# j-wilson/GPflowPILCO

Measured on AMD Instinct MI355X. Metric: moment_matched_rollout_step_elements_per_sec, higher is better.
Workload: dtype f32; 1 GPU; C3 (BASELINE configs[2]): N=2000 d=8 D=8 H=40 fp32 drift moment-match step / closed rollout; recipe=baseline: BASELINE.md recipe: lengthscales log-U[0.3,3], GP-prior targets, fresh mu~U[0,1]^d / Sigm~; N=2000, d=8, D=8, H=40, B_per_gpu=256, B_total=256, B_this_rank=256, parallelism=dp1 over B (weak), recipe=baseline, steps_requested=418, diag_pairs=f64, offdiag_pairs=f32

## Files before the change

gpflowpilco_amd/_lib.py:

```python
from __future__ import annotations

import ctypes as C
import os

_HERE = os.path.dirname(os.path.abspath(__file__))
LIB_PATH = os.environ.get("GPFLOWPILCO_MM_LIB") or os.path.join(_HERE, "libgpflowpilco_mm.so")

MM_F32, MM_F64 = 0, 1
MM_DMAX = 32
MM_M_ALIGN = 128
MM_FULL_OUTPUT_COV = 1
MM_MODEL_UNCERTAINTY = 2
MM_FORCE_GENERIC = 4
MM_STAGE_DIAG = 8
MM_STAGE_OFFDIAG = 16
MM_STAGE_FINALIZE = 32
MM_FORCE_WORST_TIER = 64
MM_WORKSPACE_CURRENT = 128
MM_FORCE_ROUTE = 256
MM_NO_ROUTE = 512
MM_SUMS_CURRENT = 1024

ERRORS = {
    -1: "MM_E_ARG: NULL pointer or non-positive size",
    -2: "MM_E_DIM: input dimension d exceeds MM_DMAX=32 or unsupported shape",
    -3: "MM_E_DTYPE: dtype must be MM_F32 or MM_F64",
    -4: "MM_E_WORKSPACE: workspace/packed buffer too small",
    -5: "MM_E_NO_C: model_uncertainty requested but the model was packed without C",
    -6: "MM_E_STATE: Euler update / closed rollout needs d == L and a full output covariance",
}

SIGNATURES = {
    "mm_abi_version": (C.c_int, []),
    "mm_packed_model_bytes": (C.c_size_t, [C.c_int] * 5),
    "mm_pack_model": (C.c_int, [C.c_void_p, C.c_size_t, C.c_int, C.c_int, C.c_int, C.c_int]
                      + [C.c_void_p] * 6 + [C.c_void_p]),
    "mm_pack_perm": (C.c_int, [C.c_void_p, C.c_size_t, C.c_int, C.c_int, C.c_int, C.c_int, C.c_void_p, C.c_void_p]),
    "mm_workspace_bytes": (C.c_size_t, [C.c_int] * 6),
    "mm_moment_match": (C.c_int, [C.c_void_p, C.c_size_t, C.c_int, C.c_int, C.c_int, C.c_int, C.c_int,
                                  C.c_void_p, C.c_void_p, C.c_int, C.c_double,
                                  C.c_void_p, C.c_void_p, C.c_void_p,
                                  C.c_void_p, C.c_size_t, C.c_void_p, C.c_void_p]),
    "mm_q_forward": (C.c_int, [C.c_void_p, C.c_size_t, C.c_int, C.c_int, C.c_int, C.c_int, C.c_int,
                               C.c_void_p, C.c_void_p, C.c_int,
                               C.c_void_p, C.c_void_p, C.c_void_p,
                               C.c_void_p, C.c_size_t, C.c_void_p, C.c_void_p]),
    "mm_Q_reduce_forward": (C.c_int, [C.c_void_p, C.c_size_t, C.c_int, C.c_int, C.c_int, C.c_int, C.c_int,
                                      C.c_int, C.c_double, C.c_void_p,
                                      C.c_void_p, C.c_size_t, C.c_void_p]),
    "mm_euler_update": (C.c_int, [C.c_int, C.c_int, C.c_int, C.c_double] + [C.c_void_p] * 8),
    "mm_expected_cost": (C.c_int, [C.c_int, C.c_int, C.c_int] + [C.c_void_p] * 6),
    "mm_offdiag_stats": (C.c_int, [C.c_void_p, C.c_size_t, C.c_int, C.c_int, C.c_int, C.c_int, C.c_int, C.c_int,
                                   C.c_void_p, C.c_size_t, C.c_void_p, C.c_void_p]),
    "mm_route_estimates": (C.c_int, [C.c_void_p, C.c_size_t, C.c_int, C.c_int, C.c_int, C.c_int, C.c_int, C.c_int,
                                     C.c_void_p, C.c_size_t, C.c_void_p, C.c_void_p]),
    "mm_compose_workspace_bytes": (C.c_size_t, [C.c_int] * 4),
    "mm_rollout_composed": (C.c_int, [C.c_void_p, C.c_size_t, C.c_int, C.c_int, C.c_int,
                                      C.c_void_p, C.c_size_t, C.c_int, C.c_int,
                                      C.c_int, C.c_int, C.c_int, C.c_double, C.c_int, C.c_int, C.POINTER(C.c_int32),
                                      C.c_double, C.c_double, C.c_void_p, C.c_void_p,
                                      C.c_void_p, C.c_void_p, C.c_void_p, C.c_void_p, C.c_void_p,
                                      C.c_void_p, C.c_size_t, C.c_void_p, C.c_size_t, C.c_void_p, C.c_size_t,
                                      C.c_void_p, C.c_void_p]),
    "mm_compose_nd_workspace_bytes": (C.c_size_t, [C.c_int] * 5),
    "mm_rollout_composed_nd": (C.c_int, [C.c_void_p, C.c_size_t, C.c_int, C.c_int, C.c_int,
                                         C.c_void_p, C.c_size_t, C.c_int, C.c_int,
                                         C.c_int, C.c_int, C.c_int, C.c_double, C.c_int, C.c_int, C.POINTER(C.c_int32),
                                         C.c_int, C.POINTER(C.c_double), C.POINTER(C.c_double), C.c_void_p, C.c_void_p,
                                         C.c_void_p, C.c_void_p, C.c_void_p, C.c_void_p, C.c_void_p,
                                         C.c_void_p, C.c_size_t, C.c_void_p, C.c_size_t, C.c_void_p, C.c_size_t,
                                         C.c_void_p, C.c_void_p]),
    "mm_compose_tape_bytes": (C.c_size_t, [C.c_int] * 6),
    "mm_rollout_composed_taped": (C.c_int, [C.c_void_p, C.c_size_t, C.c_int, C.c_int, C.c_int,
                                            C.c_void_p, C.c_size_t, C.c_int, C.c_int,
                                            C.c_int, C.c_int, C.c_int, C.c_double, C.c_int, C.c_int, C.POINTER(C.c_int32),
                                            C.c_double, C.c_double, C.c_void_p, C.c_void_p,
                                            C.c_void_p, C.c_void_p, C.c_void_p,
                                            C.c_void_p, C.c_size_t, C.c_void_p, C.c_size_t, C.c_void_p, C.c_size_t,
                                            C.c_void_p, C.c_void_p]),
    "mm_compose_backward_workspace_bytes": (C.c_size_t, [C.c_int] * 4),
    "mm_policy_grad_bytes": (C.c_size_t, [C.c_int] * 3),
    "mm_rollout_composed_backward": (C.c_int, [C.c_void_p, C.c_size_t, C.c_int, C.c_int, C.c_int,
                                               C.c_void_p, C.c_size_t, C.c_int, C.c_int,
                                               C.c_int, C.c_int, C.c_int, C.c_double, C.c_int, C.c_int, C.POINTER(C.c_int32),
                                               C.c_double, C.c_double, C.c_void_p, C.c_void_p,
                                               C.c_void_p, C.c_size_t, C.c_void_p,
                                               C.c_void_p, C.c_void_p, C.c_void_p,
                                               C.c_void_p, C.c_size_t, C.c_void_p, C.c_size_t,
# ... 99 lines not shown
```

gpflowpilco_amd/csrc/mm_common.h:

```cpp
#pragma once
#include <stddef.h>
#include <stdint.h>
#include "../../include/gpflowpilco_mm.h"

static inline size_t mm_align_up(size_t x, size_t a) { return (x + a - 1) / a * a; }
static inline int mm_round_up_int(int x, int a) { return (x + a - 1) / a * a; }
static inline size_t mm_elem_size(int dtype) { return dtype == MM_F64 ? 8 : 4; }

#define MM_ISTAGE_NO_ROUTE (1 << 20)
#define MM_ISTAGE_ROUTE (1 << 21)
#define MM_ISTAGE_NO_M56 (1 << 22)
#define MM_ISTAGE_OLD_OFFDIAG (1 << 23)
#define MM_ISTAGE_OLD_SPOLY56 (1 << 24)

static inline int mm_num_pairs(int L, int flags) {
  return (flags & MM_FULL_OUTPUT_COV) ? L * (L + 1) / 2 : L;
}

static inline int mm_moment_deg(int d) { return d <= 8 ? 4 : 2; }
static inline long long mm_binom(int n, int k) {
  if (k < 0 || k > n) return 0;
  long long r = 1;
  for (int i = 1; i <= k; ++i) r = r * (n - k + i) / i;
  return r;
}
static inline int mm_mono_count(int n, int d) { return (int)mm_binom(d + n - 1, n); }
static inline int mm_mono_offset(int n, int d) { int o = 0; for (int m = 0; m < n; ++m) o += mm_mono_count(m, d); return o; }
static inline size_t mm_rank_table_entries(int d) {
  const int dk = d <= 8 ? 8 : 32, deg = mm_moment_deg(d);
  size_t n = 0, p = 1;
  for (int k = 1; k <= deg; ++k) { p *= dk; n += p; }
  return n;
}
static inline int mm_moment_cols(int d) { return mm_round_up_int(mm_mono_offset(mm_moment_deg(d) + 1, d), 16); }
static inline int mm_moment56_off5(int d) { return d <= 8 ? mm_round_up_int(mm_mono_count(4, d), 128) : 0; }
static inline int mm_moment56_off6(int d) { return d <= 8 ? mm_moment56_off5(d) + mm_round_up_int(mm_mono_count(5, d), 128) : 0; }
static inline int mm_moment56_cols(int d) { return d <= 8 ? mm_moment56_off6(d) + mm_round_up_int(mm_mono_count(6, d), 128) : 0; }
struct MMTab56 { int ins[6], last[6], n_i16, mult2, mult3, n_f32; size_t bytes; };
static inline MMTab56 mm_tab56(int d) {
  MMTab56 t;
  int o = 0;
  for (int m = 0; m < 6; ++m) { t.ins[m] = o; o += mm_mono_count(m, d) * 8; }
  for (int k = 0; k < 6; ++k) { t.last[k] = o; o += mm_mono_count(k, d); }
  t.n_i16 = mm_round_up_int(o, 8);
  t.mult2 = 0; t.mult3 = mm_mono_count(2, d); t.n_f32 = mm_mono_count(2, d) + mm_mono_count(3, d);
  t.bytes = (size_t)t.n_i16 * 2 + (size_t)t.n_f32 * 4;
// ... 223 lines not shown
```

gpflowpilco_amd/csrc/mm_moments.hip:

```cpp
#include <hip/hip_runtime.h>
#include <math.h>
#include "mm_common.h"
#include "mm_mono.h"

typedef double f64x4m __attribute__((ext_vector_type(4)));

#define MM_GEMM_RB 64
#define MM_GEMM_NB 128
#define MM_GEMM_KB 32
#define MM_GEMM_AS 34
#define MM_GEMM_BS 144

__device__ __forceinline__ void mm_decode_pair_m(int p, int L, int& a, int& a2) {
  int r = p - L, i = 0;
  while (r >= L - 1 - i) { r -= L - 1 - i; ++i; }
  a = i; a2 = i + 1 + r;
}

__global__ __launch_bounds__(256) __attribute__((amdgpu_waves_per_eu(2, 2))) void k_wmom_gemm(const double* __restrict__ whR, const double* __restrict__ whC,
                                                      const double* __restrict__ Zm, int KMp, int L, int Mp, int B, int Po,
                                                      int nrb, int ncb, int nwork, int col_deg3,
                                                      const unsigned int* __restrict__ amaxc, const double* __restrict__ zmax2,
                                                      const int* __restrict__ gperm, double* __restrict__ mom) {
  const int orig = blockIdx.x;
// ... 285 lines not shown
      const int nsz = ksz >> LB;
      for (int idx = tid; idx < nsz; idx += 256) {
        double s = 0.0;
#pragma unroll
        for (int l = 0; l < DK; ++l) s = fma(cur[MM_PADI(l * nsz + idx)], dmu[l], s);
        oth[MM_PADI(idx)] = s;
      }
      __syncthreads();
      double* tsw = cur; cur = oth; oth = tsw;
      ksz = nsz;
      sign_binom = -sign_binom * (double)k / (double)(n - k + 1);
    }
    __syncthreads();
  }
  const double tot = mm_block_sum256m(total, red);
  if (tid == 0) s12[(size_t)b * Po + po] = tot + nh[0] * qh[0];
#undef MM_PADI
}

int mm_launch_wmom_full(const char* packed, const MMModelLayout& ml, char* ws, const MMWorkspaceLayout& wl,
                        int B, int L, int d, hipStream_t stream) {
  const int nrb = ((L - 1) * B + MM_GEMM_RB - 1) / MM_GEMM_RB, ncb = (ml.KMp + MM_GEMM_NB - 1) / MM_GEMM_NB;
  const long long nwork_ll = (long long)L * ncb * MM_MOM_SPLIT * nrb;
  if (nwork_ll <= 0 || nwork_ll > 0x7fffffffLL) return MM_E_DIM;
  hipLaunchKernelGGL(k_wmom_gemm, dim3((int)nwork_ll), dim3(256), 0, stream, (const double*)(ws + wl.whR),
                     (const double*)(ws + wl.whC), (const double*)(packed + ml.Zm), ml.KMp, L, wl.Mp, B, wl.Po, nrb, ncb,
                     (int)nwork_ll, 0x7fffffff , (const unsigned int*)nullptr, (const double*)(packed + ml.zmax2),
                     (const int*)nullptr, (double*)(ws + wl.mom));
  hipError_t e = hipGetLastError();
  return e == hipSuccess ? 0 : (int)e;
}

int mm_launch_moments56(const char* packed, const MMModelLayout& ml, char* ws, const MMWorkspaceLayout& wl,
                        int B, int L, int d, int allow, int old_spoly56, hipStream_t stream);

int mm_launch_moments(const char* packed, const MMModelLayout& ml, char* ws, const MMWorkspaceLayout& wl,
                      int B, int L, int d, const void* mu_f32, int flags, hipStream_t stream) {
  const double* Zm = (const double*)(packed + ml.Zm);
  double* mom = (double*)(ws + wl.mom);
  const int deg = mm_moment_deg(d) >= 4 ? 3 : mm_moment_deg(d);
  const int ncol_fwd = mm_mono_offset(deg + 1, d);
  const int nrb = ((L - 1) * B + MM_GEMM_RB - 1) / MM_GEMM_RB, ncb = (ncol_fwd + MM_GEMM_NB - 1) / MM_GEMM_NB;
  const long long nwork_ll = (long long)L * ncb * MM_MOM_SPLIT * nrb;
  if (nwork_ll <= 0 || nwork_ll > 0x7fffffffLL) return MM_E_DIM;
  const int nwork = (int)nwork_ll;
  const int allow = (flags & (MM_FORCE_WORST_TIER | MM_ISTAGE_NO_M56)) ? 0 : 1;
  const int col_deg3 = mm_mono_offset(3, d);
  const bool some = allow && mm_moment_deg(d) >= 4;
  if (some) {
    hipLaunchKernelGGL(k_wmom_perm, dim3(L), dim3(1024), 0, stream, (const unsigned int*)(ws + wl.amaxc),
                       (const double*)(packed + ml.zmax2), L, B, wl.Po, (int*)(ws + wl.gperm));
    hipError_t ep = hipGetLastError();
    if (ep != hipSuccess) return (int)ep;
  }
  hipLaunchKernelGGL(k_wmom_gemm, dim3(nwork), dim3(256), 0, stream, (const double*)(ws + wl.whR),
                     (const double*)(ws + wl.whC), Zm, ml.KMp, L, wl.Mp, B, wl.Po, nrb, ncb, nwork, col_deg3,
                     some ? (const unsigned int*)(ws + wl.amaxc) : (const unsigned int*)nullptr,
                     (const double*)(packed + ml.zmax2), some ? (const int*)(ws + wl.gperm) : (const int*)nullptr, mom);
  hipError_t e = hipGetLastError();
  if (e != hipSuccess) return (int)e;
  const int off1 = mm_mono_offset(1, d), off2 = mm_mono_offset(2, d), off3 = mm_mono_offset(3, d), off4 = mm_mono_offset(4, d);
#define MM_SPOLY(DK_, LB_)                                                                                                       \
  do {                                                                                                                          \
    const int dn_ = 1 << (LB_ * deg);                                                                                           \
    const int up_ = dn_ >> LB_;                                                                                                 \
    const size_t shm_ = (size_t)(dn_ + (dn_ >> 5) + up_ + (up_ >> 5) + 2 * ml.KMp + DK_ * DK_ + DK_ + 8) * sizeof(double);      \
    hipLaunchKernelGGL((k_spoly<DK_, LB_>), dim3(wl.Po, B), dim3(256), shm_, stream, (const double*)mom, ml.KMp,                \
                       (const double*)(ws + wl.pairmat), (const double*)(packed + ml.zbar), (const double*)(packed + ml.zmax2), \
                       (const unsigned int*)(ws + wl.amax), (const unsigned int*)(ws + wl.amaxc), (const float*)mu_f32, L, d, wl.P, deg, allow, off1, off2, off3, off4, \
                       (const short*)(packed + ml.rtab),                                                                        \
                       (double)MM_C6_C0, (double)MM_C6_C1, (double*)(ws + wl.s12));                                             \
  } while (0)
  if (d <= 8) MM_SPOLY(8, 3); else MM_SPOLY(32, 5);
#undef MM_SPOLY
  e = hipGetLastError();
  if (e != hipSuccess) return (int)e;
  if (flags & MM_ISTAGE_NO_M56) {
    if (mm_moment56_cols(d) <= 0 || wl.Po <= 0) return 0;
    const hipError_t em = hipMemsetAsync(ws + wl.s56, 0xFF, (size_t)B * wl.Po * sizeof(double), stream);
    if (em != hipSuccess) return (int)em;
    const hipError_t es = hipMemsetAsync(ws + wl.estS, 0, (size_t)B * wl.Po * sizeof(float), stream);
    return es == hipSuccess ? 0 : (int)es;
  }
  return mm_launch_moments56(packed, ml, ws, wl, B, L, d, some ? 1 : 0, (flags & MM_ISTAGE_OLD_SPOLY56) ? 1 : 0, stream);
}

__global__ void k_offdiag_stats(const unsigned int* __restrict__ amax, const double* __restrict__ zmax2,
                                const unsigned char* __restrict__ gflag, int ng, int L, int Po, int n,
                                int32_t* __restrict__ out) {
  const int idx = blockIdx.x * blockDim.x + threadIdx.x;
  bool c = false, in = false, part = false;
  int groups = 0;
  if (idx < n) {
    int a, a2;
    mm_decode_pair_m(L + idx % Po, L, a, a2);
    const float b2 = mm_collapse_bound2(amax[idx], zmax2[a2]);
    c = b2 <= MM_COLLAPSE_BOUND2;
    in = b2 <= MM_INSIDE_BOUND2;
    part = !c && mm_item_collapsed(amax[n + idx]);
    for (int g = 0; g < ng; ++g) groups += gflag[(size_t)idx * ng + g] ? 1 : 0;
  }
  const unsigned long long m = __ballot(c), mi = __ballot(in), mp = __ballot(part);
  if ((threadIdx.x & 63) == 0 && m) atomicAdd(out, (int)__popcll(m));
  if ((threadIdx.x & 63) == 0 && mi) atomicAdd(out + 2, (int)__popcll(mi));
  if ((threadIdx.x & 63) == 0 && mp) atomicAdd(out + 4, (int)__popcll(mp));
#pragma unroll
  for (int off = 32; off > 0; off >>= 1) groups += __shfl_down(groups, off, 64);
  if ((threadIdx.x & 63) == 0 && groups) atomicAdd(out + 5, groups);
  if (idx == 0) out[1] = n;
}

extern "C" int mm_offdiag_stats(const void* packed, size_t packed_bytes, int L, int M, int d, int dtype, int B, int flags,
                                const void* workspace, size_t workspace_bytes, int32_t* out, void* stream) {
  if (!packed || !workspace || !out || L <= 0 || M <= 0 || d <= 0 || d > MM_DMAX || B <= 0) return MM_E_ARG;
  const MMModelLayout ml = mm_model_layout(L, M, d, dtype, 1);
  const MMWorkspaceLayout wl = mm_workspace_layout(B, L, M, d, dtype, flags);
  if (packed_bytes < ml.Cm || workspace_bytes < wl.total) return MM_E_WORKSPACE;
// ... 16 lines not shown
```

gpflowpilco_amd/csrc/mm_moments6.hip:

```cpp
#include <hip/hip_runtime.h>
#include <math.h>
#include "mm_common.h"
#include "mm_mono.h"
#include "mm_f32_tile.h"
#include <atomic>
#include <type_traits>

__device__ __forceinline__ void mm6_decode_pair_o(int lp, int L, int& a, int& a2) {
  int r = lp, i = 0;
  while (r >= L - 1 - i) { r -= L - 1 - i; ++i; }
  a = i; a2 = i + 1 + r;
}

__global__ __launch_bounds__(256) void k_pack_zm56(char* packed, MMModelLayout lay, int L, int M, int d, int N56p,
                                                   const double* __restrict__ Z) {
  const int c = blockIdx.x, a = blockIdx.y, tid = threadIdx.x;
  const int n4 = mm_binom_i(d + 3, 4), n5 = mm_binom_i(d + 4, 5), n6 = mm_binom_i(d + 5, 6);
  const int off5 = ((n4 + 127) / 128) * 128;
  const int off6 = off5 + ((n5 + 127) / 128) * 128;
  const double* zbar = (const double*)(packed + lay.zbar) + (size_t)a * d;
  unsigned short* oh = (unsigned short*)(packed + lay.Zm56) + (((size_t)a * 2 + 0) * N56p + c) * lay.Mp;
  unsigned short* om = (unsigned short*)(packed + lay.Zm56) + (((size_t)a * 2 + 1) * N56p + c) * lay.Mp;
  int n = 0, k[6] = {0, 0, 0, 0, 0, 0};
  if (c < n4) { n = 4; mm_mono_unrank(c, 4, k); }
// ... 147 lines not shown
#pragma unroll
    for (int ks = 0; ks < 2; ++ks) {
      const int ch = ((ks * 2 + h) ^ swz) * 16;
      bf16x8 Ah[2], Am[2], Th[2], Tm[2];
#pragma unroll
      for (int t = 0; t < 2; ++t) {
        Ah[t] = *reinterpret_cast<const bf16x8*>(base + fragA[t] + ch);
        Am[t] = *reinterpret_cast<const bf16x8*>(base + 8192 + fragA[t] + ch);
        Th[t] = *reinterpret_cast<const bf16x8*>(base + fragB[t] + ch);
        Tm[t] = *reinterpret_cast<const bf16x8*>(base + 8192 + fragB[t] + ch);
      }
#pragma unroll
      for (int rt = 0; rt < 2; ++rt)
#pragma unroll
        for (int ct = 0; ct < 2; ++ct) {
          acc[rt][ct] = __builtin_amdgcn_mfma_f32_32x32x16_bf16(Am[rt], Th[ct], acc[rt][ct], 0, 0, 0);
          acc[rt][ct] = __builtin_amdgcn_mfma_f32_32x32x16_bf16(Ah[rt], Tm[ct], acc[rt][ct], 0, 0, 0);
          acc[rt][ct] = __builtin_amdgcn_mfma_f32_32x32x16_bf16(Ah[rt], Th[ct], acc[rt][ct], 0, 0, 0);
        }
    }
  }
#pragma unroll
  for (int rt = 0; rt < 2; ++rt)
#pragma unroll
    for (int e = 0; e < 16; ++e) {
      const int item = orow[wr * 64 + rt * 32 + 8 * (e >> 2) + 4 * h + (e & 3)];
      if (item < 0) continue;
      float* o = mom56 + (size_t)item * N56p + (size_t)cb * MM6_TB + wc * 64 + l31;
#pragma unroll
      for (int ct = 0; ct < 2; ++ct) o[ct * 32] = acc[rt][ct][e];
    }
}

#ifndef MM6_THREADS
#define MM6_THREADS 768
#endif
#define MM6_WAVES (MM6_THREADS / 64)
#ifndef MM6_NC
#define MM6_NC 2
#endif
template <int K, bool TRANSG, int MODE, int NC = MM6_NC, int NW = MM6_WAVES>
__device__ __forceinline__ void mm6_step(const float* __restrict__ Tin, int nJin, int nI, float* __restrict__ Tout, int nJp,
                                         const short* __restrict__ ins, int d, const float (&G)[64], const float* __restrict__ multJ,
                                         int xs, float& acc, int wave, int lane) {
  const int chunks = (nJp + 64 * NC - 1) / (64 * NC);
  auto dots = [&](auto i0c, const float (&v)[NC][8], float (&s)[NC][8]) __attribute__((always_inline)) {
    constexpr int I0 = decltype(i0c)::value;
#pragma unroll
    for (int q = 0; q < NC; ++q)
#pragma unroll
      for (int i = I0; i < 8; ++i) s[q][i] = G[0 * 8 + i] * v[q][0];
#pragma unroll
    for (int j = 1; j < 8; ++j)
#pragma unroll
      for (int q = 0; q < NC; ++q)
#pragma unroll
        for (int i = I0; i < 8; ++i) s[q][i] = fmaf(G[j * 8 + i], v[q][j], s[q][i]);
  };
  auto body = [&](int I, int t, const int (&Jp)[NC], const bool (&jv)[NC], const int (&off)[NC][8], const float (&mj)[NC]) __attribute__((always_inline)) {
    const float* tin = Tin + I * nJin;
    float v[NC][8], s[NC][8];
#pragma unroll
    for (int q = 0; q < NC; ++q)
#pragma unroll
      for (int j = 0; j < 8; ++j) v[q][j] = tin[off[q][j]];
    if (t < 4) dots(std::integral_constant<int, 0>{}, v, s);
// ... 450 lines not shown
        G[4 * q] = g4.x; G[4 * q + 1] = g4.y; G[4 * q + 2] = g4.z; G[4 * q + 3] = g4.w;
      }
    };
    float acc4 = 0.0f, dummy = 0.0f;
    const float* Q4 = nq + sy[4];
    const float* N4 = nq;
    load_G(1);
    mm6_do<D8, 0, false, 0, NC0, NW, 4, 0>(Q4, Bf4, sy, tabi, tb, d, G, nullptr, 0, dummy, wave, lane);
    __syncthreads();
    mm6_do<D8, 1, false, 1, 1, NW, 3, 37>(Bf4, X4, sy, tabi, tb, d, G, mult2, xs4, dummy, wave, lane);
    __syncthreads();
    load_G(0);
    mm6_do<D8, 0, true, 0, NC0, NW, 4, 0>(N4, Bf4, sy, tabi, tb, d, G, nullptr, 0, dummy, wave, lane);
    __syncthreads();
    mm6_do<D8, 1, true, 2, 1, NW, 3, 37>(Bf4, X4, sy, tabi, tb, d, G, nullptr, xs4, acc4, wave, lane);
    double tot = (double)MM_C6_C1 * (double)acc4;
#pragma unroll
    for (int off = 32; off > 0; off >>= 1) {
      tot += __shfl_down(tot, off, 64); s2r += __shfl_down(s2r, off, 64); s2c += __shfl_down(s2c, off, 64);
    }
    if (lane == 0) { redd[wave * 3 + 0] = tot; redd[wave * 3 + 1] = s2r; redd[wave * 3 + 2] = s2c; }
    __syncthreads();
    if (tid == 0) {
      double t = 0.0, r2 = 0.0, c2 = 0.0;
      for (int w = 0; w < NW; ++w) { t += redd[w * 3]; r2 += redd[w * 3 + 1]; c2 += redd[w * 3 + 2]; }
      s56[item] = t;
      estS[item] = mm6_estS(bound2, false, false, r2, c2);
    }
    __syncthreads();
  }
}

int mm_launch_moments56(const char* packed, const MMModelLayout& ml, char* ws, const MMWorkspaceLayout& wl,
                        int B, int L, int d, int allow, int old_spoly56, hipStream_t stream) {
  const int N56p = mm_moment56_cols(d);
  if (N56p <= 0 || wl.Po <= 0) return 0;
  if (allow) {
    const int nrb = ((L - 1) * B + MM6_TB - 1) / MM6_TB, ncb = N56p / MM6_TB;
    const long long nwork_ll = (long long)L * ncb * nrb;
    if (nwork_ll <= 0 || nwork_ll > 0x7fffffffLL) return MM_E_DIM;
    if ((size_t)B * wl.Po * 4 * wl.Mp >= 0xffffffffull || (size_t)L * 2 * N56p * wl.Mp >= 0xffffffffull) return MM_E_DIM;
    const size_t shm = 2 * MM6_STAGE_BYTES + MM6_TB * sizeof(int);
    static std::atomic<unsigned long long> attr_done{0ull};
    int dev = 0;
    if (hipGetDevice(&dev) != hipSuccess) dev = 64;
    const unsigned long long bit = (dev >= 0 && dev < 64) ? (1ull << dev) : 0ull;
    if (!bit || !(attr_done.load() & bit)) {
      const hipError_t ea = hipFuncSetAttribute((const void*)k_wmom56_gemm, hipFuncAttributeMaxDynamicSharedMemorySize, (int)shm);
      if (ea != hipSuccess) return (int)ea;
      attr_done.fetch_or(bit);
    }
    hipLaunchKernelGGL(k_wmom56_gemm, dim3((int)nwork_ll), dim3(256), shm, stream, (const unsigned short*)(ws + wl.wsp),
                       (const unsigned short*)(packed + ml.Zm56), N56p, L, wl.Mp, B, wl.Po, nrb, ncb, (int)nwork_ll,
                       mm_moment56_off5(d) / MM6_TB, mm_moment56_off6(d) / MM6_TB,
                       (const int*)(ws + wl.gperm), (float*)(ws + wl.mom56));
    hipError_t e = hipGetLastError();
    if (e != hipSuccess) return (int)e;
  }
  const int nitem = B * wl.Po;
  int* ilist = (int*)(ws + wl.ilist);
  {
    const hipError_t em = hipMemsetAsync(ilist, 0, 16, stream);
    if (em != hipSuccess) return (int)em;
  }
  hipLaunchKernelGGL(k_item_classes, dim3((nitem + 255) / 256), dim3(256), 0, stream, (const unsigned int*)(ws + wl.amaxc),
                     (const double*)(packed + ml.zmax2), L, wl.Po, nitem, allow, ilist, (double*)(ws + wl.s56), (float*)(ws + wl.estS));
  {
    const hipError_t ec = hipGetLastError();
    if (ec != hipSuccess) return (int)ec;
  }
  if (!allow) return 0;
  int sy[7];
  for (int k = 0; k < 7; ++k) sy[k] = mm_mono_count(k, d);
  size_t nfl = (size_t)2 * (sy[4] + sy[5] + sy[6]) + (size_t)sy[3] * (sy[3] + 1) + (size_t)sy[2] * sy[4] + (size_t)sy[1] * sy[5] + 6 * MM6_WAVES + 128 + 16
               + (size_t)sy[1] * sy[3] + (size_t)sy[2] * (sy[2] + 1);
  nfl = (nfl + 1) & ~(size_t)1;
  const size_t shm = nfl * sizeof(float);
  static std::atomic<unsigned long long> attr2_done{0ull};
  static std::atomic<int> ncu_cached[64];
  int dev = 0;
  if (hipGetDevice(&dev) != hipSuccess) dev = 64;
  const unsigned long long bit2 = (dev >= 0 && dev < 64) ? (1ull << dev) : 0ull;
  int ncu = bit2 ? ncu_cached[dev].load() : 0;
  if (!bit2 || !(attr2_done.load() & bit2)) {
    hipError_t ea = hipFuncSetAttribute((const void*)k_spoly56<false>, hipFuncAttributeMaxDynamicSharedMemorySize, 160 * 1024);
// ... 28 lines not shown
```

gpflowpilco_amd/csrc/mm_route.hip:

```cpp
#include <hip/hip_runtime.h>
#include <math.h>
#include "mm_common.h"
#include "mm_fork.h"
#include "mm_mono.h"
#include "mm_adjoint.h"

__device__ __forceinline__ void mmx_decode_pair_o(int lp, int L, int& a, int& a2) {
  int r = lp, i = 0;
  while (r >= L - 1 - i) { r -= L - 1 - i; ++i; }
  a = i; a2 = i + 1 + r;
}

__device__ __forceinline__ double mmx_est(double e2, unsigned int, double) {
  return 5.9604644775390625e-8 * (2.0 / 3.0) * sqrt(e2);
}

__global__ __launch_bounds__(64) void k_route_decide(const float* __restrict__ estO, int npanel, const double* __restrict__ s12,
                                                     const double* __restrict__ f1raw, const unsigned int* __restrict__ amax,
                                                     const double* __restrict__ zmax2, int L, int Po, double tol, int force,
                                                     int* __restrict__ rlist, int* __restrict__ rcount, int* __restrict__ rflag,
                                                     int slot, int32_t* __restrict__ status, const float* __restrict__ estS) {
  const int b = blockIdx.x, lane = threadIdx.x;
  auto zmax2a2 = [&](int po) { int a, a2; mmx_decode_pair_o(po, L, a, a2); return zmax2[a2]; };
  double sc = 0.0;
// ... 44 lines not shown
  for (int po = lane; po < Po; po += 64) {
    int a, a2;
    mmx_decode_pair_o(po, L, a, a2);
    const double v = fabs(s12[(size_t)b * Po + po] - f1raw[(size_t)b * L + a] * f1raw[(size_t)b * L + a2]);
    sc = v > sc ? v : sc;
  }
#pragma unroll
  for (int off = 32; off > 0; off >>= 1) { const double o = __shfl_xor(sc, off, 64); sc = o > sc ? o : sc; }
  for (int po = lane; po < Po; po += 64) {
    const float* e = estO + ((size_t)b * Po + po) * npanel;
    double e2 = 0.0;
    for (int pn = 0; pn < npanel; ++pn) e2 += (double)e[pn];
    if (estS) e2 += (double)estS[(size_t)b * Po + po];
    out[((size_t)b * Po + po) * 2 + 0] = mmx_est(e2, amax[(size_t)b * Po + po], zmax2a2(po));
    out[((size_t)b * Po + po) * 2 + 1] = sc;
  }
}

extern "C" int mm_route_estimates(const void* packed, size_t packed_bytes, int L, int M, int d, int dtype, int B, int flags,
                                  const void* workspace, size_t workspace_bytes, double* out, void* stream) {
  if (!packed || !workspace || !out || L <= 0 || M <= 0 || d <= 0 || d > MM_DMAX || B <= 0) return MM_E_ARG;
  if (dtype != MM_F32) return MM_E_DTYPE;
  const MMWorkspaceLayout wl = mm_workspace_layout(B, L, M, d, dtype, flags);
  const MMModelLayout ml = mm_model_layout(L, M, d, dtype, 1);
  if (workspace_bytes < wl.total || packed_bytes < ml.Cm) return MM_E_WORKSPACE;
  if (wl.Po <= 0) return 0;
  const char* ws = (const char*)workspace;
  if (const int rj = mm_fork_join_wait((hipStream_t)stream)) return rj;
  hipLaunchKernelGGL(k_route_report, dim3(B), dim3(64), 0, (hipStream_t)stream, (const float*)(ws + wl.estO),
                     (wl.Mp + MM_PANEL_ROWS - 1) / MM_PANEL_ROWS, (const double*)(ws + wl.s12), (const double*)(ws + wl.f1raw),
                     (const unsigned int*)(ws + wl.amax), (const double*)((const char*)packed + ml.zmax2), L, wl.Po, out,
                     d <= 8 ? (const float*)(ws + wl.estS) : (const float*)nullptr);
  hipError_t e = hipGetLastError();
  return e == hipSuccess ? 0 : (int)e;
}

__device__ __forceinline__ double mmx_rem(double x) {
  if (fabs(x) < 0.5) {
    double p = 4.7794773323873853e-14;
    p = fma(p, x, 7.6471637318198165e-13);
    p = fma(p, x, 1.1470745597729725e-11);
    p = fma(p, x, 1.6059043836821613e-10);
    p = fma(p, x, 2.08767569878681e-09);
    p = fma(p, x, 2.505210838544172e-08);
    p = fma(p, x, 2.755731922398589e-07);
    p = fma(p, x, 2.7557319223985893e-06);
    p = fma(p, x, 2.48015873015873e-05);
    p = fma(p, x, 1.984126984126984e-04);
    p = fma(p, x, 1.388888888888889e-03);
    p = fma(p, x, 8.333333333333333e-03);
    p = fma(p, x, 4.1666666666666664e-02);
    p = fma(p, x, 1.6666666666666666e-01);
    return (x * x) * (x * p);
  }
  return expm1(x) - fma(0.5 * x, x, x);
}

__device__ __forceinline__ double mmx_wave_sum(double v) {
#pragma unroll
  for (int off = 32; off > 0; off >>= 1) v += __shfl_xor(v, off, 64);
  return v;
}

template <int DK, bool AGG>
__global__ __launch_bounds__(256) void k_route_f64(const int* __restrict__ rlist, const int* __restrict__ rcount,
                                                   const double* __restrict__ Zt64, const double* __restrict__ Zc64, int Kz,
// ... 176 lines not shown
```

gpflowpilco_amd/ops.py:

```python
from __future__ import annotations

from dataclasses import dataclass, field
from typing import Dict, Optional, Tuple

import torch

from . import _lib
from ._lib import (MM_F32, MM_F64, MM_FORCE_GENERIC, MM_FULL_OUTPUT_COV, MM_WORKSPACE_CURRENT, MM_SUMS_CURRENT,
                   MM_MODEL_UNCERTAINTY, check, lib)

_DTYPES = {torch.float32: MM_F32, torch.float64: MM_F64}


def _dtype_code(dtype: torch.dtype) -> int:
  try:
    return _DTYPES[dtype]
  except KeyError:
    raise TypeError(f"moment matching supports float32/float64 states, got {dtype}") from None


def _ptr(t: Optional[torch.Tensor]):
  return None if t is None else t.data_ptr()


def _require_device(*tensors: torch.Tensor):
  for t in tensors:
    if t is not None and not t.is_cuda:
      raise RuntimeError("gpflowpilco_amd kernels run on the GPU only (no CPU fallback): "
                         f"got a tensor on {t.device}")


def _stream(device) -> int:
  return torch.cuda.current_stream(device).cuda_stream

# ... 172 lines not shown
  return c, n, inside


def offdiag_row_groups(pm: PackedModel, B: int, flags: int):
  ws = pm.workspace(B, flags, peek=True)
  out = torch.zeros(6, dtype=torch.int32, device=pm.device)
  rc = lib().mm_offdiag_stats(pm.buf.data_ptr(), pm.nbytes, pm.L, pm.M, pm.d, _dtype_code(pm.dtype), B, flags,
                              ws.data_ptr(), ws.numel(), out.data_ptr(), _stream(pm.device))
  check(rc, "mm_offdiag_stats")
  o = out.tolist()
  Mp = (pm.M + _lib.MM_M_ALIGN - 1) // _lib.MM_M_ALIGN * _lib.MM_M_ALIGN
  return o[4], o[5], o[1] * (Mp // 64)


def offdiag_routed(pm: PackedModel, B: int, flags: int) -> int:
  if pm.dtype != torch.float32 or pm.L < 2 or not (flags & MM_FULL_OUTPUT_COV):
    return 0
  ws = pm.workspace(B, flags, peek=True)
  out = torch.zeros(6, dtype=torch.int32, device=pm.device)
  rc = lib().mm_offdiag_stats(pm.buf.data_ptr(), pm.nbytes, pm.L, pm.M, pm.d, _dtype_code(pm.dtype), B, flags,
                              ws.data_ptr(), ws.numel(), out.data_ptr(), _stream(pm.device))
  check(rc, "mm_offdiag_stats")
  return int(out[3])


def route_estimates(pm: PackedModel, B: int, flags: int) -> torch.Tensor:
  Po = pm.L * (pm.L - 1) // 2 if (flags & MM_FULL_OUTPUT_COV) else 0
  out = torch.zeros(B, Po, 2, dtype=torch.float64, device=pm.device)
  if Po:
    ws = pm.workspace(B, flags, peek=True)
    rc = lib().mm_route_estimates(pm.buf.data_ptr(), pm.nbytes, pm.L, pm.M, pm.d, _dtype_code(pm.dtype), B, flags,
                                  ws.data_ptr(), ws.numel(), out.data_ptr(), _stream(pm.device))
    check(rc, "mm_route_estimates")
  return out


def euler_update(mu, Sigma, f1, Sff, cross_pre, dt: float = 1.0):
  _require_device(mu, Sigma, f1, Sff, cross_pre)
  B, d = mu.shape
  if f1.shape != (B, d) or Sff.shape != (B, d, d) or cross_pre.shape != (B, d, d):
    raise ValueError("euler_update needs d == L and a full output covariance")
  args = [t.contiguous() for t in (mu, Sigma, f1, Sff, cross_pre)]
  mu_o, S_o = torch.empty_like(args[0]), torch.empty_like(args[1])
  rc = lib().mm_euler_update(B, d, _dtype_code(mu.dtype), float(dt), *[t.data_ptr() for t in args],
                             mu_o.data_ptr(), S_o.data_ptr(), _stream(mu.device))
  check(rc, "mm_euler_update")
  return mu_o, S_o


def rollout_closed(pm: PackedModel, mu: torch.Tensor, Sigma: torch.Tensor, num_steps: int,
                   dt: float = 1.0, model_uncertainty: bool = True, jitter: float = 0.0,
                   keep_trajectory: bool = False, force_generic: bool = False):
  B, mu, Sigma = _prep_state(pm, mu, Sigma)
  mu, Sigma = mu.clone(), Sigma.clone()
  flags = make_flags(True, model_uncertainty, force_generic)
  ws = pm.workspace(B, flags)
  tmu = tS = None
  if keep_trajectory:
    tmu = torch.empty(num_steps, B, pm.d, dtype=pm.dtype, device=pm.device)
    tS = torch.empty(num_steps, B, pm.d, pm.d, dtype=pm.dtype, device=pm.device)
  rc = lib().mm_rollout_closed(pm.buf.data_ptr(), pm.nbytes, pm.L, pm.M, pm.d, _dtype_code(pm.dtype), B,
                               int(num_steps), float(dt), flags, float(jitter),
                               mu.data_ptr(), Sigma.data_ptr(), _ptr(tmu), _ptr(tS),
                               ws.data_ptr(), ws.numel(), pm.status().data_ptr(), _stream(pm.device))
  check(rc, "mm_rollout_closed")
  return (mu, Sigma, tmu, tS) if keep_trajectory else (mu, Sigma)
# ... 407 lines not shown
```

include/gpflowpilco_mm.h:

```cpp
#ifndef GPFLOWPILCO_MM_H
#define GPFLOWPILCO_MM_H

#include <stddef.h>
#include <stdint.h>

#ifdef __cplusplus
extern "C" {
#endif

#define MM_F32 0
#define MM_F64 1

#define MM_DMAX 32
#define MM_M_ALIGN 128

#define MM_FULL_OUTPUT_COV   1
#define MM_MODEL_UNCERTAINTY 2
#define MM_FORCE_GENERIC     4
#define MM_STAGE_DIAG        8
#define MM_STAGE_OFFDIAG    16
#define MM_STAGE_FINALIZE   32
#define MM_FORCE_WORST_TIER 64
#define MM_WORKSPACE_CURRENT 128
#define MM_FORCE_ROUTE 256
// ... 34 lines not shown
                    void* Sff,
                    void* cross_pre,
                    void* workspace, size_t workspace_bytes,
                    int32_t* status, void* stream);

int mm_q_forward(const void* packed, size_t packed_bytes, int L, int M, int d, int dtype, int B,
                 const void* mu, const void* Sigma, int flags,
                 void* f1, void* cross_pre, void* q_out,
                 void* workspace, size_t workspace_bytes, int32_t* status, void* stream);

int mm_Q_reduce_forward(const void* packed, size_t packed_bytes, int L, int M, int d, int dtype, int B,
                        int flags, double jitter, void* Sff,
                        void* workspace, size_t workspace_bytes, void* stream);

int mm_euler_update(int B, int d, int dtype, double dt,
                    const void* mu, const void* Sigma,
                    const void* f1, const void* Sff, const void* cross_pre,
                    void* mu_out, void* Sigma_out, void* stream);

int mm_rollout_closed(const void* packed, size_t packed_bytes, int L, int M, int d, int dtype, int B, int H,
                      double dt, int flags, double jitter,
                      void* mu, void* Sigma, void* traj_mu, void* traj_Sigma,
                      void* workspace, size_t workspace_bytes,
                      int32_t* status, void* stream);

int mm_expected_cost(int N, int d, int dtype, const void* mean, const void* cov,
                     const void* target, const void* precis, void* cost, void* stream);

int mm_offdiag_stats(const void* packed, size_t packed_bytes, int L, int M, int d, int dtype, int B, int flags,
                     const void* workspace, size_t workspace_bytes, int32_t* out, void* stream);

int mm_route_estimates(const void* packed, size_t packed_bytes, int L, int M, int d, int dtype, int B, int flags,
                       const void* workspace, size_t workspace_bytes, double* out, void* stream);

size_t mm_compose_workspace_bytes(int B, int nx, int na, int dtype);
int mm_rollout_composed(const void* drift_packed, size_t drift_bytes, int drift_L, int drift_M, int drift_d,
                        const void* policy_packed, size_t policy_bytes, int policy_M, int policy_d,
                        int dtype, int B, int H, double dt, int nx, int na, const int32_t* active_dims,
                        double head_scale, double head_shift, const void* target, const void* precis,
                        void* mx, void* Sxx, void* cost, void* traj_mu, void* traj_Sigma,
                        void* ws_drift, size_t ws_drift_bytes, void* ws_policy, size_t ws_policy_bytes,
                        void* ws_compose, size_t ws_compose_bytes, int32_t* status, void* stream);

size_t mm_compose_nd_workspace_bytes(int B, int nx, int na, int nu, int dtype);
int mm_rollout_composed_nd(const void* drift_packed, size_t drift_bytes, int drift_L, int drift_M, int drift_d,
                           const void* policy_packed, size_t policy_bytes, int policy_M, int policy_d,
                           int dtype, int B, int H, double dt, int nx, int na, const int32_t* active_dims,
                           int nu, const double* head_scale, const double* head_shift,
                           const void* target, const void* precis,
                           void* mx, void* Sxx, void* cost, void* traj_mu, void* traj_Sigma,
                           void* ws_drift, size_t ws_drift_bytes, void* ws_policy, size_t ws_policy_bytes,
                           void* ws_compose, size_t ws_compose_bytes, int32_t* status, void* stream);

size_t mm_compose_tape_bytes(int B, int H, int nx, int na, int drift_M, int dtype);
int mm_rollout_composed_taped(const void* drift_packed, size_t drift_bytes, int drift_L, int drift_M, int drift_d,
                              const void* policy_packed, size_t policy_bytes, int policy_M, int policy_d,
                              int dtype, int B, int H, double dt, int nx, int na, const int32_t* active_dims,
                              double head_scale, double head_shift, const void* target, const void* precis,
                              void* mx, void* Sxx, void* cost, void* ws_drift, size_t ws_drift_bytes,
                              void* ws_policy, size_t ws_policy_bytes, void* tape, size_t tape_bytes,
                              int32_t* status, void* stream);

size_t mm_compose_backward_workspace_bytes(int B, int nx, int na, int drift_M);
size_t mm_policy_grad_bytes(int B, int policy_M, int policy_d);
int mm_rollout_composed_backward(const void* drift_packed, size_t drift_bytes, int drift_L, int drift_M, int drift_d,
                                 const void* policy_packed, size_t policy_bytes, int policy_M, int policy_d,
// ... 109 lines not shown
```

Baseline: 42420 rollout step-elements/s (B*H per rollout second).

## Add warp-specialized triple-buffered ring kernel for degree-5/6 moment GEMM

```diff
diff --git a/gpflowpilco_amd/_lib.py b/gpflowpilco_amd/_lib.py
--- a/gpflowpilco_amd/_lib.py
+++ b/gpflowpilco_amd/_lib.py
@@ -54,6 +54,8 @@
                                    C.c_void_p, C.c_size_t, C.c_void_p, C.c_void_p]),
     "mm_route_estimates": (C.c_int, [C.c_void_p, C.c_size_t, C.c_int, C.c_int, C.c_int, C.c_int, C.c_int, C.c_int,
                                      C.c_void_p, C.c_size_t, C.c_void_p, C.c_void_p]),
+    "mm_moments56_read": (C.c_int, [C.c_void_p, C.c_size_t, C.c_int, C.c_int, C.c_int, C.c_int, C.c_int, C.c_int,
+                                    C.c_void_p, C.c_size_t, C.c_void_p, C.c_void_p]),
     "mm_compose_workspace_bytes": (C.c_size_t, [C.c_int] * 4),
     "mm_rollout_composed": (C.c_int, [C.c_void_p, C.c_size_t, C.c_int, C.c_int, C.c_int,
                                       C.c_void_p, C.c_size_t, C.c_int, C.c_int,
diff --git a/gpflowpilco_amd/csrc/mm_common.h b/gpflowpilco_amd/csrc/mm_common.h
--- a/gpflowpilco_amd/csrc/mm_common.h
+++ b/gpflowpilco_amd/csrc/mm_common.h
@@ -12,6 +12,7 @@
 #define MM_ISTAGE_NO_M56 (1 << 22)
 #define MM_ISTAGE_OLD_OFFDIAG (1 << 23)
 #define MM_ISTAGE_OLD_SPOLY56 (1 << 24)
+#define MM_ISTAGE_OLD_WMOM56 (1 << 25)
 
 static inline int mm_num_pairs(int L, int flags) {
   return (flags & MM_FULL_OUTPUT_COV) ? L * (L + 1) / 2 : L;
diff --git a/gpflowpilco_amd/csrc/mm_moments.hip b/gpflowpilco_amd/csrc/mm_moments.hip
--- a/gpflowpilco_amd/csrc/mm_moments.hip
+++ b/gpflowpilco_amd/csrc/mm_moments.hip
@@ -341,7 +341,7 @@
 }
 
 int mm_launch_moments56(const char* packed, const MMModelLayout& ml, char* ws, const MMWorkspaceLayout& wl,
-                        int B, int L, int d, int allow, int old_spoly56, hipStream_t stream);
+                        int B, int L, int d, int allow, int old_spoly56, int old_wmom56, hipStream_t stream);
 
 int mm_launch_moments(const char* packed, const MMModelLayout& ml, char* ws, const MMWorkspaceLayout& wl,
                       int B, int L, int d, const void* mu_f32, int flags, hipStream_t stream) {
@@ -391,7 +391,8 @@
     const hipError_t es = hipMemsetAsync(ws + wl.estS, 0, (size_t)B * wl.Po * sizeof(float), stream);
     return es == hipSuccess ? 0 : (int)es;
   }
-  return mm_launch_moments56(packed, ml, ws, wl, B, L, d, some ? 1 : 0, (flags & MM_ISTAGE_OLD_SPOLY56) ? 1 : 0, stream);
+  return mm_launch_moments56(packed, ml, ws, wl, B, L, d, some ? 1 : 0, (flags & MM_ISTAGE_OLD_SPOLY56) ? 1 : 0,
+                             (flags & MM_ISTAGE_OLD_WMOM56) ? 1 : 0, stream);
 }
 
 __global__ void k_offdiag_stats(const unsigned int* __restrict__ amax, const double* __restrict__ zmax2,
diff --git a/gpflowpilco_amd/csrc/mm_moments6.hip b/gpflowpilco_amd/csrc/mm_moments6.hip
--- a/gpflowpilco_amd/csrc/mm_moments6.hip
+++ b/gpflowpilco_amd/csrc/mm_moments6.hip
@@ -203,6 +203,145 @@
     }
 }
 
+#define MM6R_TM 256
+#define MM6R_STAGES 3
+#define MM6R_STAGE_BYTES 49152
+#define MM6R_B_OFF 32768
+#define MM6R_CWAVES 8
+#define MM6R_LWAVES 4
+#define MM6R_THREADS ((MM6R_CWAVES + MM6R_LWAVES) * 64)
+
+__global__ __launch_bounds__(MM6R_THREADS) void k_wmom56_gemm_ring(const unsigned short* __restrict__ wsp, const unsigned short* __restrict__ Zm56,
+                                                                   int N56p, int L, int Mp, int B, int Po, int nrb, int ncb, int nwork, int cb5, int cb6,
+                                                                   const int* __restrict__ gperm, float* __restrict__ mom56) {
+  const int orig = blockIdx.x;
+  const int xcd = orig & 7, slot = orig >> 3;
+  const int qn = nwork >> 3, rn = nwork & 7;
+  int wi = (xcd < rn ? xcd * (qn + 1) : rn * (qn + 1) + (xcd - rn) * qn) + slot;
+  const int rb = wi % nrb; wi /= nrb;
+  const int cb = wi % ncb; wi /= ncb;
+  const int a = wi;
+  const int R = (L - 1) * B;
+  const int ncoll = gperm[(size_t)L * R + (cb < cb5 ? 0 : (cb < cb6 ? 1 : 2)) * L + a];
+  if (rb * MM6R_TM >= ncoll) return;
+  const int* perm = gperm + (size_t)a * R;
+  extern __shared__ __align__(1024) char lds[];
+  int* orow = reinterpret_cast<int*>(lds + MM6R_STAGES * MM6R_STAGE_BYTES);
+  const int tid = threadIdx.x, wv = __builtin_amdgcn_readfirstlane(tid >> 6), lane = tid & 63, l31 = lane & 31, h = lane >> 5;
+  auto row_item = [&](int r) {
+    const int which = r / B, b = r - which * B;
+    const int ap = which < a ? which : which + 1;
+    const int lo = ap < a ? ap : a, hi = ap < a ? a : ap;
+    const int po = lo * (L - 1) - lo * (lo - 1) / 2 + (hi - lo - 1);
+    return ((b * Po + po) << 1) | (ap < a ? 1 : 0);
+  };
+  if (tid < MM6R_TM) {
+    const int r = rb * MM6R_TM + tid;
+    orow[tid] = r < ncoll ? row_item(perm[r]) : -1;
+  }
+  const int nkb = Mp / MM6_KB;
+  if (wv >= MM6R_CWAVES) {
+    const int sq = wv - MM6R_CWAVES;
+    unsigned int srcA[2][4], srcB[2][2];
+    const int lc = ((lane & 3) ^ ((lane >> 4) & 3)) * 8;
+#pragma unroll
+    for (int i = 0; i < 4; ++i) {
+      int r = rb * MM6R_TM + sq * 64 + i * 16 + (lane >> 2);
+      r = r < ncoll ? r : ncoll - 1;
+      const size_t it = (size_t)row_item(perm[r]) * 2;
+      srcA[0][i] = (unsigned int)(it * Mp) + lc;
+      srcA[1][i] = (unsigned int)((it + 1) * Mp) + lc;
+    }
+#pragma unroll
+    for (int i = 0; i < 2; ++i) {
+      const int row = sq * 32 + i * 16 + (lane >> 2);
+#pragma unroll
+      for (int part = 0; part < 2; ++part)
+        srcB[part][i] = (unsigned int)((((size_t)a * 2 + part) * N56p + (size_t)cb * MM6_TB + row) * Mp) + lc;
+    }
+    auto stage = [&](int kb, int buf) {
+      char* dA = lds + buf * MM6R_STAGE_BYTES + sq * 4096;
+      char* dB = lds + buf * MM6R_STAGE_BYTES + MM6R_B_OFF + sq * 2048;
+#pragma unroll
+      for (int part = 0; part < 2; ++part) {
+#pragma unroll
+        for (int i = 0; i < 4; ++i)
+          __builtin_amdgcn_global_load_lds((const __attribute__((address_space(1))) void*)(wsp + srcA[part][i] + kb * MM6_KB),
+                                           (__attribute__((address_space(3))) void*)(dA + part * 16384 + i * 1024), 16, 0, 0);
+#pragma unroll
+        for (int i = 0; i < 2; ++i)
+          __builtin_amdgcn_global_load_lds((const __attribute__((address_space(1))) void*)(Zm56 + srcB[part][i] + kb * MM6_KB),
+                                           (__attribute__((address_space(3))) void*)(dB + part * 8192 + i * 1024), 16, 0, 0);
+      }
+    };
+    stage(0, 0);
+    if (nkb > 1) stage(1, 1);
+    int cur = 0;
+    for (int kb = 0; kb < nkb; ++kb) {
+      if (kb + 1 < nkb) __builtin_amdgcn_s_waitcnt(0x007c);
+      else __builtin_amdgcn_s_waitcnt(0x0070);
+      __builtin_amdgcn_s_barrier();
+      if (kb + 2 < nkb) stage(kb + 2, cur == 0 ? 2 : cur - 1);
+      cur = cur == 2 ? 0 : cur + 1;
+    }
+    return;
+  }
+  const int wr = wv >> 1, wc = wv & 1;
+  f32x16 acc[2][2];
+#pragma unroll
+  for (int rt = 0; rt < 2; ++rt)
+#pragma unroll
+    for (int ct = 0; ct < 2; ++ct)
+#pragma unroll
+      for (int e = 0; e < 16; ++e) acc[rt][ct][e] = 0.0f;
+  int fragA[2], fragB[2];
+#pragma unroll
+  for (int t = 0; t < 2; ++t) {
+    fragA[t] = (wr * 64 + t * 32 + l31) * 64;
+    fragB[t] = MM6R_B_OFF + (wc * 64 + t * 32 + l31) * 64;
+  }
+  const int swz = (l31 >> 2) & 3;
+  int cur = 0;
+  for (int kb = 0; kb < nkb; ++kb) {
+    __builtin_amdgcn_s_waitcnt(0xc07f);
+    __builtin_amdgcn_s_barrier();
+    const char* base = lds + cur * MM6R_STAGE_BYTES;
+    bf16x8 Ah[2][2], Am[2][2], Th[2][2], Tm[2][2];
+#pragma unroll
+    for (int ks = 0; ks < 2; ++ks) {
+      const int ch = ((ks * 2 + h) ^ swz) * 16;
+#pragma unroll
+      for (int t = 0; t < 2; ++t) {
+        Ah[ks][t] = *reinterpret_cast<const bf16x8*>(base + fragA[t] + ch);
+        Am[ks][t] = *reinterpret_cast<const bf16x8*>(base + 16384 + fragA[t] + ch);
+        Th[ks][t] = *reinterpret_cast<const bf16x8*>(base + fragB[t] + ch);
+        Tm[ks][t] = *reinterpret_cast<const bf16x8*>(base + 8192 + fragB[t] + ch);
+      }
+    }
+#pragma unroll
+    for (int ks = 0; ks < 2; ++ks)
+#pragma unroll
+      for (int rt = 0; rt < 2; ++rt)
+#pragma unroll
+        for (int ct = 0; ct < 2; ++ct) {
+          acc[rt][ct] = __builtin_amdgcn_mfma_f32_32x32x16_bf16(Am[ks][rt], Th[ks][ct], acc[rt][ct], 0, 0, 0);
+          acc[rt][ct] = __builtin_amdgcn_mfma_f32_32x32x16_bf16(Ah[ks][rt], Tm[ks][ct], acc[rt][ct], 0, 0, 0);
+          acc[rt][ct] = __builtin_amdgcn_mfma_f32_32x32x16_bf16(Ah[ks][rt], Th[ks][ct], acc[rt][ct], 0, 0, 0);
+        }
+    cur = cur == 2 ? 0 : cur + 1;
+  }
+#pragma unroll
+  for (int rt = 0; rt < 2; ++rt)
+#pragma unroll
+    for (int e = 0; e < 16; ++e) {
+      const int item = orow[wr * 64 + rt * 32 + 8 * (e >> 2) + 4 * h + (e & 3)];
+      if (item < 0) continue;
+      float* o = mom56 + (size_t)item * N56p + (size_t)cb * MM6_TB + wc * 64 + l31;
+#pragma unroll
+      for (int ct = 0; ct < 2; ++ct) o[ct * 32] = acc[rt][ct][e];
+    }
+}
+
 #ifndef MM6_THREADS
 #define MM6_THREADS 768
 #endif
@@ -719,25 +858,30 @@
 }
 
 int mm_launch_moments56(const char* packed, const MMModelLayout& ml, char* ws, const MMWorkspaceLayout& wl,
-                        int B, int L, int d, int allow, int old_spoly56, hipStream_t stream) {
+                        int B, int L, int d, int allow, int old_spoly56, int old_wmom56, hipStream_t stream) {
   const int N56p = mm_moment56_cols(d);
   if (N56p <= 0 || wl.Po <= 0) return 0;
   if (allow) {
-    const int nrb = ((L - 1) * B + MM6_TB - 1) / MM6_TB, ncb = N56p / MM6_TB;
+    const int tm = old_wmom56 ? MM6_TB : MM6R_TM;
+    const int nrb = ((L - 1) * B + tm - 1) / tm, ncb = N56p / MM6_TB;
     const long long nwork_ll = (long long)L * ncb * nrb;
     if (nwork_ll <= 0 || nwork_ll > 0x7fffffffLL) return MM_E_DIM;
     if ((size_t)B * wl.Po * 4 * wl.Mp >= 0xffffffffull || (size_t)L * 2 * N56p * wl.Mp >= 0xffffffffull) return MM_E_DIM;
-    const size_t shm = 2 * MM6_STAGE_BYTES + MM6_TB * sizeof(int);
+    const size_t shm_old = 2 * MM6_STAGE_BYTES + MM6_TB * sizeof(int);
+    const size_t shm_ring = MM6R_STAGES * MM6R_STAGE_BYTES + MM6R_TM * sizeof(int);
+    const size_t shm = old_wmom56 ? shm_old : shm_ring;
     static std::atomic<unsigned long long> attr_done{0ull};
     int dev = 0;
     if (hipGetDevice(&dev) != hipSuccess) dev = 64;
     const unsigned long long bit = (dev >= 0 && dev < 64) ? (1ull << dev) : 0ull;
     if (!bit || !(attr_done.load() & bit)) {
-      const hipError_t ea = hipFuncSetAttribute((const void*)k_wmom56_gemm, hipFuncAttributeMaxDynamicSharedMemorySize, (int)shm);
+      hipError_t ea = hipFuncSetAttribute((const void*)k_wmom56_gemm, hipFuncAttributeMaxDynamicSharedMemorySize, (int)shm_old);
+      if (ea == hipSuccess) ea = hipFuncSetAttribute((const void*)k_wmom56_gemm_ring, hipFuncAttributeMaxDynamicSharedMemorySize, (int)shm_ring);
       if (ea != hipSuccess) return (int)ea;
       attr_done.fetch_or(bit);
     }
-    hipLaunchKernelGGL(k_wmom56_gemm, dim3((int)nwork_ll), dim3(256), shm, stream, (const unsigned short*)(ws + wl.wsp),
+    hipLaunchKernelGGL((old_wmom56 ? k_wmom56_gemm : k_wmom56_gemm_ring), dim3((int)nwork_ll), dim3(old_wmom56 ? 256 : MM6R_THREADS), shm, stream,
+                       (const unsigned short*)(ws + wl.wsp),
                        (const unsigned short*)(packed + ml.Zm56), N56p, L, wl.Mp, B, wl.Po, nrb, ncb, (int)nwork_ll,
                        mm_moment56_off5(d) / MM6_TB, mm_moment56_off6(d) / MM6_TB,
                        (const int*)(ws + wl.gperm), (float*)(ws + wl.mom56));
diff --git a/gpflowpilco_amd/csrc/mm_route.hip b/gpflowpilco_amd/csrc/mm_route.hip
--- a/gpflowpilco_amd/csrc/mm_route.hip
+++ b/gpflowpilco_amd/csrc/mm_route.hip
@@ -100,6 +100,21 @@
                      (const unsigned int*)(ws + wl.amax), (const double*)((const char*)packed + ml.zmax2), L, wl.Po, out,
                      d <= 8 ? (const float*)(ws + wl.estS) : (const float*)nullptr);
   hipError_t e = hipGetLastError();
+  return e == hipSuccess ? 0 : (int)e;
+}
+
+extern "C" int mm_moments56_read(const void* packed, size_t packed_bytes, int L, int M, int d, int dtype, int B, int flags,
+                                 const void* workspace, size_t workspace_bytes, float* out, void* stream) {
+  if (!packed || !workspace || !out || L <= 0 || M <= 0 || d <= 0 || d > MM_DMAX || B <= 0) return MM_E_ARG;
+  if (dtype != MM_F32) return MM_E_DTYPE;
+  if (mm_moment56_cols(d) <= 0) return MM_E_DIM;
+  const MMWorkspaceLayout wl = mm_workspace_layout(B, L, M, d, dtype, flags);
+  const MMModelLayout ml = mm_model_layout(L, M, d, dtype, 1);
+  if (workspace_bytes < wl.total || packed_bytes < ml.Cm) return MM_E_WORKSPACE;
+  if (wl.Po <= 0) return 0;
+  if (const int rj = mm_fork_join_wait((hipStream_t)stream)) return rj;
+  const hipError_t e = hipMemcpyAsync(out, (const char*)workspace + wl.mom56, (size_t)B * wl.Po * 2 * mm_moment56_cols(d) * sizeof(float),
+                                      hipMemcpyDeviceToDevice, (hipStream_t)stream);
   return e == hipSuccess ? 0 : (int)e;
 }
 
diff --git a/gpflowpilco_amd/ops.py b/gpflowpilco_amd/ops.py
--- a/gpflowpilco_amd/ops.py
+++ b/gpflowpilco_amd/ops.py
@@ -1,5 +1,6 @@
 from __future__ import annotations
 
+import math
 from dataclasses import dataclass, field
 from typing import Dict, Optional, Tuple
 
@@ -238,6 +239,19 @@
     rc = lib().mm_route_estimates(pm.buf.data_ptr(), pm.nbytes, pm.L, pm.M, pm.d, _dtype_code(pm.dtype), B, flags,
                                   ws.data_ptr(), ws.numel(), out.data_ptr(), _stream(pm.device))
     check(rc, "mm_route_estimates")
+  return out
+
+
+def moments56_read(pm: PackedModel, B: int, flags: int) -> torch.Tensor:
+  Po = pm.L * (pm.L - 1) // 2 if (flags & MM_FULL_OUTPUT_COV) else 0
+  n = [math.comb(pm.d + k - 1, k) for k in (4, 5, 6)]
+  N56p = sum((c + 127) // 128 * 128 for c in n)
+  out = torch.zeros(B, Po, 2, N56p, dtype=torch.float32, device=pm.device)
+  if Po:
+    ws = pm.workspace(B, flags, peek=True)
+    rc = lib().mm_moments56_read(pm.buf.data_ptr(), pm.nbytes, pm.L, pm.M, pm.d, _dtype_code(pm.dtype), B, flags,
+                                 ws.data_ptr(), ws.numel(), out.data_ptr(), _stream(pm.device))
+    check(rc, "mm_moments56_read")
   return out
 
 
diff --git a/include/gpflowpilco_mm.h b/include/gpflowpilco_mm.h
--- a/include/gpflowpilco_mm.h
+++ b/include/gpflowpilco_mm.h
@@ -90,6 +90,9 @@
 
 int mm_route_estimates(const void* packed, size_t packed_bytes, int L, int M, int d, int dtype, int B, int flags,
                        const void* workspace, size_t workspace_bytes, double* out, void* stream);
+
+int mm_moments56_read(const void* packed, size_t packed_bytes, int L, int M, int d, int dtype, int B, int flags,
+                      const void* workspace, size_t workspace_bytes, float* out, void* stream);
 
 size_t mm_compose_workspace_bytes(int B, int nx, int na, int dtype);
 int mm_rollout_composed(const void* drift_packed, size_t drift_bytes, int drift_L, int drift_M, int drift_d,
```

Measured after the change: 42460 rollout step-elements/s (B*H per rollout second), median of 2. Within noise of the previous version (+0.1%).
